# 2892931976/consensus-rs

Measured on AMD Instinct MI355X. Metric: BFT instance-rounds/sec (whole node), N=64 f=21, 1/2/4/8 GPUs; bit-exact, higher is better.
Workload: dtype u64

## Files before the change

### consensus-rs_amd/csrc/bft_common.h

```cpp
#pragma once
#include <stdint.h>

#if defined(__HIPCC__)
#include <hip/hip_runtime.h>
#define BFT_FN __host__ __device__ inline
#else
#define BFT_FN inline
#endif

namespace bft {

struct Params {
    uint32_t n;
    uint32_t seg;
    uint32_t heights;
    uint32_t hcap;
    uint32_t max_ticks;
    uint32_t block_period;
    uint64_t genesis_time;
    uint64_t seed;
    uint32_t thr16;
    uint32_t byz_count;
    uint32_t crash_thr32;
    uint32_t crash_on;
    uint32_t phase_cap;
    uint32_t need_seed;
    uint64_t silent_mask[4];
    uint32_t first_instance;
    uint32_t n_instances;
    uint32_t genesis_seed;
    uint32_t fast;
    const uint8_t* addresses;
    const uint8_t* genesis_hash;
    uint32_t* committed_height;
    uint32_t* flags;
    uint32_t* ticks;
    uint64_t* views;
    uint32_t* rec;
    uint8_t* hash;
    uint64_t* trace;
    uint32_t trace_ticks;
    uint32_t pad1;
    uint64_t* stamps;
    uint64_t* hist;
    uint32_t window_mask;
    uint32_t rows;
    uint32_t* rcs;
    uint32_t q;
    uint32_t nmask;
    uint32_t* resume_flags;
    uint32_t* resume_q;
    uint32_t* resume_hint;
    uint32_t* save;
    uint64_t save_stride;
    uint32_t resume_mode;
    uint32_t seed_le;
    uint32_t backlog_replay;
    uint32_t pad3;
    uint32_t* backlog;
    uint32_t* mlog;
    uint32_t* mlog_n;
    uint32_t mlog_cap;
    uint32_t pad4;
    uint64_t forged[4];
    uint32_t* vsnap;
    uint32_t* votes;
    uint32_t* sfx;
    uint32_t sfx_x0, sfx_rows;
    uint32_t chain_prio;
    uint32_t rcs_k;
    uint32_t* spec;
    uint32_t chain_mode;
    uint32_t chain_grid;
    uint32_t chain_inline;
};
constexpr uint32_t RCS_DEFAULT_K = 16, RCS_MAX_K = 4096;
constexpr uint32_t MLOG_WORDS = 8;
constexpr uint32_t MLOG_FORGED = 1u, MLOG_WILD = 2u, MLOG_EQUIV = 4u, MLOG_OLD = 8u;

constexpr uint32_t FLAG_SAFETY = 1u, FLAG_PHASE_CAP = 2u, FLAG_CORE_PANIC = 4u, FLAG_OUTBOX = 8u,
                   FLAG_TIMEOUT = 16u, FLAG_RCS_OVERFLOW = 32u, FLAG_WINDOW = 64u;
constexpr uint32_t HIST_BINS = 130;
constexpr int NSTAMP = 18;

constexpr uint32_t ST_ACCEPT_REQUEST = 1, ST_PREPREPARED = 2, ST_PREPARED = 3, ST_COMMITTED = 4;

constexpr int MT_PREPREPARE = 1, MT_PREPARE = 2, MT_COMMIT = 3, MT_ROUND_CHANGE = 4;
constexpr int CM_OK = 0, CM_UNKNOWN = 1, CM_FUTURE_BLOCK = 2, CM_OLD = 3, CM_FUTURE_MSG = 4;
BFT_FN int check_message_class(int code, uint32_t vh, uint32_t h, uint32_t st) {
    if (vh == 0) return CM_UNKNOWN;
    if (code == MT_ROUND_CHANGE) { if (vh > h) return CM_FUTURE_BLOCK; if (vh < h) return CM_OLD; return CM_OK; }
    if (vh > h) return CM_FUTURE_BLOCK;
    if (vh < h) return CM_OLD;
    if (st == ST_ACCEPT_REQUEST) return code > MT_PREPREPARE ? CM_FUTURE_MSG : CM_OK;
    return CM_OK;
}

constexpr uint64_t BLK_NONE = 0;
constexpr uint64_t BLK_VALID = 1ull << 34;
constexpr uint64_t BLK_ID_MASK = (1ull << 35) - 1;
constexpr uint64_t BLK_HP_MASK = (1ull << 33) - 1;
BFT_FN uint64_t blk_make(uint32_t h, uint32_t prop, uint32_t var, uint32_t T) {
    return (uint64_t)(h & 0xffffffu) | ((uint64_t)(prop & 0x1ffu) << 24) | ((uint64_t)(var & 1u) << 33) |
           BLK_VALID | ((uint64_t)T << 35);
}
BFT_FN bool blk_valid(uint64_t b) { return (b & BLK_VALID) != 0; }
BFT_FN uint32_t blk_h(uint64_t b) { return (uint32_t)(b & 0xffffffu); }
BFT_FN uint32_t blk_prop(uint64_t b) { return (uint32_t)((b >> 24) & 0x1ffu); }
BFT_FN uint32_t blk_var(uint64_t b) { return (uint32_t)((b >> 33) & 1u); }
BFT_FN uint32_t blk_T(uint64_t b) { return (uint32_t)(b >> 35); }
BFT_FN bool blk_eq(uint64_t a, uint64_t b) {
    return blk_valid(a) && blk_valid(b) && ((a ^ b) & BLK_ID_MASK) == 0;
}
BFT_FN uint32_t blk_d32(uint64_t b) {
    if (!blk_valid(b)) return 0;
    return (uint32_t)(b & 0x3fffffu) | (blk_prop(b) << 22) | (blk_var(b) << 30) | 0x80000000u;
}
BFT_FN bool digest_match(uint64_t d, bool wild, uint64_t t) {
    if (!blk_valid(d) || !blk_valid(t)) return false;
    if (((d ^ t) & BLK_HP_MASK) != 0) return false;
    return wild || blk_var(d) == blk_var(t);
}

template <int NW>
struct Bits {
    uint64_t w[NW];
    BFT_FN static Bits zero() { Bits b; for (int k = 0; k < NW; ++k) b.w[k] = 0; return b; }
    BFT_FN static Bits from(uint64_t x) { Bits b = zero(); b.w[0] = x; return b; }
    BFT_FN static Bits from(const Bits& x) { return x; }
    BFT_FN static Bits low(uint32_t n) {
        if (NW == 1) { Bits b; b.w[0] = n >= 64u ? ~0ull : ((1ull << n) - 1ull); return b; }
        Bits b;
        for (int k = 0; k < NW; ++k) {
            uint32_t lo = 64u * (uint32_t)k;
            b.w[k] = n >= lo + 64u ? ~0ull : (n <= lo ? 0ull : ((1ull << (n - lo)) - 1ull));
        }
        return b;
    }
    BFT_FN static Bits bit(uint32_t i) {
        Bits b;
        for (int k = 0; k < NW; ++k) b.w[k] = ((i >> 6) == (uint32_t)k) ? (1ull << (i & 63u)) : 0ull;
        return b;
    }
    BFT_FN uint64_t word(int i) const {
        uint64_t x = 0;
        for (int k = 0; k < NW; ++k) x = (i == k) ? w[k] : x;
        return x;
    }
    BFT_FN bool get(uint32_t i) const { return (word((int)(i >> 6)) >> (i & 63u)) & 1ull; }
    BFT_FN void set(uint32_t i) {
        const uint64_t b = 1ull << (i & 63u);
        for (int k = 0; k < NW; ++k) w[k] |= ((i >> 6) == (uint32_t)k) ? b : 0ull;
    }
    BFT_FN bool any() const { uint64_t x = 0; for (int k = 0; k < NW; ++k) x |= w[k]; return x != 0; }
    BFT_FN bool none() const { return !any(); }
    BFT_FN uint32_t popc() const {
        uint32_t c = 0;
        for (int k = 0; k < NW; ++k) c += (uint32_t)__builtin_popcountll(w[k]);
// ... 664 lines not shown
```

### consensus-rs_amd/csrc/bftsim.hip

```cpp
#include <hip/hip_runtime.h>

#include <stdio.h>
#include <stdlib.h>
#include <string.h>

#include <dlfcn.h>
#include <unistd.h>
#include <rccl/rccl.h>
#include <hipcub/hipcub.hpp>

#include <mutex>
#include <string>
#include <utility>
#include <vector>

#include "bft_hip.h"
#include "bft_fast64.h"
#include "bft_crypto.h"
#include "bft_trace.h"
#include "bft_twins.h"
#include "bft_audit.h"
#include "bft_archive.h"
#include "bft_ledger.h"

// ... 583 lines not shown
                       (uint32_t*)(h->d_evict + EVICT_BYTES / 16));
    return hipGetLastError();
}

static void use_set0_scratch(bftsim* h) {
    if (h->n_sets == 0 || !h->sets[0].hist) return;
    bftsim::RowSet& r = h->sets[0];
    h->d_hist = r.hist; h->d_rcs = r.rcs; h->d_backlog = r.backlog; h->d_resume = r.resume; h->d_save = r.save;
    h->d_resume_q = r.resume_q;
}

static void trace_drop(bftsim* h) {
    if (!h->d_tkeep && !h->d_tfoff && h->trace_n == 0) return;
    (void)hipFree(h->d_tkeep); (void)hipFree(h->d_tfoff); (void)hipFree(h->d_twkeep);
    h->d_tkeep = nullptr; h->d_tfoff = nullptr; h->d_twkeep = nullptr; h->d_tif0 = nullptr;
    h->trace_n = h->trace_M = h->trace_F = 0;
    h->trace_has_twins = false;
    h->twin_counts[0] = h->twin_counts[1] = 0;
    h->trace_moff.clear(); h->trace_ioff.clear();
}

static int sync_all(bftsim* h);
static void free_bufs(bftsim* h) {
    trace_drop(h);
    if (h->n_pend) (void)sync_all(h);
    h->n_pend = 0;
    h->last_pipe = false;
    use_set0_scratch(h);
    if (h->n_sets == 0) {
        (void)hipFree(h->d_ch); (void)hipFree(h->d_flags); (void)hipFree(h->d_ticks); (void)hipFree(h->d_views);
        (void)hipFree(h->d_rec); (void)hipFree(h->d_hash);
    }
    for (uint32_t k = 0; k < h->n_sets; ++k) {
        bftsim::RowSet& r = h->sets[k];
        (void)hipFree(r.ch); (void)hipFree(r.flags); (void)hipFree(r.ticks); (void)hipFree(r.views);
        (void)hipFree(r.rec); (void)hipFree(r.hash); (void)hipFree(r.sfx); (void)hipFree(r.spec);
        (void)hipFree(r.byz); (void)hipFree(r.bad); (void)hipFree(r.pred);
        if (k > 0) {
            (void)hipFree(r.hist); (void)hipFree(r.rcs); (void)hipFree(r.backlog); (void)hipFree(r.resume);
            (void)hipFree(r.save); (void)hipFree(r.resume_q);
        }
        r.ch = r.flags = r.ticks = nullptr; r.views = nullptr; r.rec = nullptr; r.hash = nullptr; r.sfx = nullptr;
        r.spec = nullptr; r.byz = nullptr; r.bad = nullptr; r.pred = nullptr;
        r.hist = nullptr; r.rcs = r.backlog = r.resume = r.save = r.resume_q = nullptr;
    }

    (void)hipFree(h->d_trace); (void)hipFree(h->d_tips); (void)hipFree(h->d_rcs);
    h->d_rcs = nullptr;
    (void)hipFree(h->d_backlog);
    h->d_backlog = nullptr;
    (void)hipFree(h->d_mlog); (void)hipFree(h->d_mlog_n);
    h->d_mlog = nullptr; h->d_mlog_n = nullptr;
    (void)hipFree(h->d_vsnap); (void)hipFree(h->d_votes); (void)hipFree(h->d_vsig); (void)hipFree(h->d_vhas);
    h->d_vsnap = nullptr; h->d_votes = nullptr; h->d_vsig = nullptr; h->d_vhas = nullptr; h->vsig_n = 0;
    h->backlog_bytes = 0;
    (void)hipFree(h->d_resume); (void)hipFree(h->d_save); (void)hipFree(h->d_resume_q);
    h->d_resume = nullptr; h->d_save = nullptr; h->d_resume_q = nullptr;
    for (uint32_t k = 0; k < bftsim::MAX_SETS; ++k) h->sets[k].busy = false;
    h->n_sets = 0;
    h->cur_set = 0;
    h->d_ch = h->d_flags = h->d_ticks = nullptr; h->d_views = nullptr;
    h->d_rec = nullptr; h->d_hash = nullptr; h->d_trace = nullptr; h->d_tips = nullptr;
    h->cap_inst = 0;
    h->n_req = 0;
    h->last_n = 0;
    h->last_first = 0;
}

static int flush_batch(bftsim* h, bool final = false);
static int sync_all(bftsim* h) {
    HIPCHECK(h, hipSetDevice(h->device));
    if (int rc = flush_batch(h, true)) return rc;
    HIPCHECK(h, hipStreamSynchronize(h->last_stream));
    for (uint32_t k = 0; k < bftsim::MAX_CS; ++k)
        if (h->cs[k]) HIPCHECK(h, hipStreamSynchronize(h->cs[k]));
    for (uint32_t k = 0; k < bftsim::MAX_HS; ++k)
        if (h->hstr[k]) HIPCHECK(h, hipStreamSynchronize(h->hstr[k]));
    return BFTSIM_OK;
}

#ifdef BFT_STAMPS
static uint64_t* g_stamps = nullptr;
static uint64_t g_stamp_waves = 0;
#endif

namespace {
struct Rccl {
    ncclResult_t (*get_id)(ncclUniqueId*) = nullptr;
    ncclResult_t (*init_rank)(ncclComm_t*, int, ncclUniqueId, int) = nullptr;
    ncclResult_t (*all_reduce)(const void*, void*, size_t, ncclDataType_t, ncclRedOp_t, ncclComm_t,
                               hipStream_t) = nullptr;
    ncclResult_t (*destroy)(ncclComm_t) = nullptr;
    const char* (*err)(ncclResult_t) = nullptr;
    bool ok = false;
    std::string why;
};
Rccl& rccl() {
    static Rccl r;
    static std::once_flag once;
    std::call_once(once, [] {
        void* lib = dlopen("librccl.so.1", RTLD_NOW | RTLD_GLOBAL);
        if (!lib) lib = dlopen("/opt/rocm/lib/librccl.so.1", RTLD_NOW | RTLD_GLOBAL);
        if (!lib) { r.why = std::string("dlopen librccl.so.1: ") + dlerror(); return; }
        r.get_id = (decltype(r.get_id))dlsym(lib, "ncclGetUniqueId");
        r.init_rank = (decltype(r.init_rank))dlsym(lib, "ncclCommInitRank");
        r.all_reduce = (decltype(r.all_reduce))dlsym(lib, "ncclAllReduce");
        r.destroy = (decltype(r.destroy))dlsym(lib, "ncclCommDestroy");
        r.err = (decltype(r.err))dlsym(lib, "ncclGetErrorString");
        r.ok = r.get_id && r.init_rank && r.all_reduce && r.destroy && r.err;
        if (!r.ok) r.why = "librccl.so.1 lacks an entry point";
    });
    return r;
}
struct StdoutToStderr {
    int saved;
    StdoutToStderr() {
        fflush(stdout);
        saved = dup(1);
        if (saved >= 0) dup2(2, 1);
    }
    ~StdoutToStderr() {
        fflush(stdout);
        if (saved >= 0) { dup2(saved, 1); close(saved); }
    }
};
void comm_destroy(ncclComm_t c) {
    if (rccl().ok) (void)rccl().destroy(c);
}

struct SigApi {
    int (*create)(int, void**) = nullptr;
    void (*destroy)(void*) = nullptr;
    const char* (*last_error)(const void*) = nullptr;
    int (*secret_to_address)(void*, const uint8_t*, uint64_t, uint8_t*, uint8_t*, uint8_t*, void*) = nullptr;
    int (*sign)(void*, const uint8_t*, const uint32_t*, const uint8_t*, uint64_t, uint8_t*, uint8_t*, void*) = nullptr;
    int (*recover)(void*, const uint8_t*, const uint8_t*, uint64_t, uint8_t*, uint8_t*, uint8_t*, void*) = nullptr;
    bool ok = false;
    std::string why;
};
void sig_api_anchor() {}
SigApi& sig_api() {
    static SigApi a;
    static std::once_flag once;
    std::call_once(once, [] {
        Dl_info di;
        std::string path = "libbftsig.so";
        if (dladdr((void*)&sig_api_anchor, &di) && di.dli_fname) {
            std::string self = di.dli_fname;
            size_t k = self.rfind('/');
            if (k != std::string::npos) path = self.substr(0, k + 1) + "libbftsig.so";
        }
        void* lib = dlopen(path.c_str(), RTLD_NOW | RTLD_GLOBAL);
        if (!lib) { a.why = std::string("dlopen ") + path + ": " + dlerror(); return; }
        a.create = (decltype(a.create))dlsym(lib, "bftsig_create");
        a.destroy = (decltype(a.destroy))dlsym(lib, "bftsig_destroy");
        a.last_error = (decltype(a.last_error))dlsym(lib, "bftsig_last_error");
        a.secret_to_address = (decltype(a.secret_to_address))dlsym(lib, "bftsig_secret_to_address");
        a.sign = (decltype(a.sign))dlsym(lib, "bftsig_sign");
        a.recover = (decltype(a.recover))dlsym(lib, "bftsig_recover");
        a.ok = a.create && a.destroy && a.last_error && a.secret_to_address && a.sign && a.recover;
        if (!a.ok) a.why = path + " lacks an entry point";
    });
    return a;
}
}

extern "C" {

#ifdef BFT_STAMPS
int bftsim_debug_stamps(uint64_t* out, uint32_t cap) {
    if (!out || cap == 0) return bft::NSTAMP;
    std::vector<uint64_t> v(g_stamp_waves * bft::NSTAMP);
    if (hipDeviceSynchronize() != hipSuccess) return -2;
    if (hipMemcpy(v.data(), g_stamps, v.size() * 8, hipMemcpyDeviceToHost) != hipSuccess) return -2;
    const uint32_t m = cap < (uint32_t)bft::NSTAMP ? cap : (uint32_t)bft::NSTAMP;
    for (uint32_t k = 0; k < m; ++k) out[k] = 0;
    for (uint64_t w = 0; w < g_stamp_waves; ++w)
        for (uint32_t k = 0; k < m; ++k) out[k] += v[w * bft::NSTAMP + k];
    return bft::NSTAMP;
}
#endif

uint32_t bftsim_two_thirds_majority(uint32_t n) { return (2u * n) / 3u; }
uint32_t bftsim_seed_from_hash(const uint8_t hash[32], uint32_t n) { return n ? bft::seed_from_hash(hash, n) : 0; }
uint32_t bftsim_seed_from_hash_order(const uint8_t hash[32], uint32_t n, uint32_t order) {
    return n ? bft::seed_from_hash(hash, n, order == BFTSIM_SEED_LE) : 0;
}
uint32_t bftsim_calc_proposer(const uint8_t prev_hash[32], uint32_t n, uint64_t round) {
    if (n == 0) return 0;
    return (uint32_t)(((uint64_t)bft::seed_from_hash(prev_hash, n) + round % n) % n);
}
void bftsim_keccak256(const uint8_t* data, size_t len, uint8_t out[32]) { host_keccak(data, len, out); }
void bftsim_genesis_hash(const bftsim_config* cfg, uint8_t out[32]) { host_genesis_hash(cfg, out); }
int bftsim_check_message(uint32_t code, uint64_t msg_height, uint64_t core_height, uint32_t state) {
    if (code < 1 || code > 4 || state < 1 || state > 4 || msg_height >= (1ull << 32) || core_height >= (1ull << 32))
        return BFTSIM_EINVAL;
    return bft::check_message_class((int)code, (uint32_t)msg_height, (uint32_t)core_height, state);
}
int bftsim_view_cmp(uint64_t h1, uint64_t r1, uint64_t h2, uint64_t r2) {
    if (h1 != h2) return h1 < h2 ? -1 : 1;
    if (r1 != r2) return r1 < r2 ? -1 : 1;
    return 0;
}

const char* bftsim_last_error(bftsim_t* h) { return h ? h->err.c_str() : "null handle"; }

int bftsim_create(const bftsim_config* cfg, int hip_device, bftsim_t** out) {
    if (!cfg || !out) return BFTSIM_EINVAL;
    *out = nullptr;
    if (cfg->n < 1 || cfg->n > 256) return BFTSIM_EUNSUPPORTED;
    if (cfg->heights < 1 || cfg->heights > (1u << 20) || cfg->max_ticks < 1 || cfg->max_ticks > (1u << 28) ||
        !cfg->addresses || cfg->phase_cap < 1 || cfg->phase_cap > 255 || cfg->block_period < 1)
        return BFTSIM_EINVAL;
    for (uint32_t i = 1; i < cfg->n; ++i)
        if (memcmp(cfg->addresses + 20 * (i - 1), cfg->addresses + 20 * i, 20) >= 0) return BFTSIM_EINVAL;
    if (cfg->seed_byte_order > BFTSIM_SEED_LE || cfg->header_encoding != BFTSIM_ENC_RMP_COMPACT ||
        cfg->backlog_mode > BFTSIM_BACKLOG_REPLAY || cfg->reserved != 0)
        return BFTSIM_EINVAL;
    bftsim* h = new bftsim();
    h->cfg = *cfg;
    h->addresses.assign(cfg->addresses, cfg->addresses + 20 * cfg->n);
    h->cfg.addresses = h->addresses.data();
    h->device = hip_device;
    host_genesis_hash(&h->cfg, h->genesis_hash);
    h->genesis_seed = bft::seed_from_hash(h->genesis_hash, cfg->n, cfg->seed_byte_order == BFTSIM_SEED_LE);
    h->seg = bft::segment_size(cfg->n);
    h->hcap = cfg->heights + 64;
    *out = h;
    hipError_t e = hipSetDevice(hip_device);
    if (e != hipSuccess) return fail(h, BFTSIM_EHIP, std::string("hipSetDevice: ") + hipGetErrorString(e));
    HIPCHECK(h, hipMalloc(&h->d_addr, 20 * cfg->n));
    HIPCHECK(h, hipMemcpy(h->d_addr, h->addresses.data(), 20 * cfg->n, hipMemcpyHostToDevice));
    HIPCHECK(h, hipMalloc(&h->d_ghash, 32));
    HIPCHECK(h, hipMemcpy(h->d_ghash, h->genesis_hash, 32, hipMemcpyHostToDevice));
    HIPCHECK(h, hipMalloc(&h->d_stats, 16 * sizeof(unsigned long long)));
    HIPCHECK(h, hipMalloc(&h->d_hist, bft::HIST_BINS * sizeof(uint64_t)));
    for (uint32_t i = 0; i < bftsim::RING; ++i) {
        HIPCHECK(h, hipEventCreate(&h->ring[i].c0)); HIPCHECK(h, hipEventCreate(&h->ring[i].c1));
        HIPCHECK(h, hipEventCreate(&h->ring[i].h0)); HIPCHECK(h, hipEventCreate(&h->ring[i].h1));
        HIPCHECK(h, hipEventCreateWithFlags(&h->ring[i].sx, hipEventDisableTiming));
    }
    for (uint32_t i = 0; i < bftsim::MAX_SETS; ++i)
        HIPCHECK(h, hipEventCreateWithFlags(&h->sets[i].done, hipEventDisableTiming));
    return BFTSIM_OK;
}

void bftsim_destroy(bftsim_t* h) {
    if (!h) return;
    (void)hipSetDevice(h->device);
    free_bufs(h);
    (void)hipFree(h->d_addr); (void)hipFree(h->d_ghash); (void)hipFree(h->d_stats); (void)hipFree(h->d_hist);
    (void)hipFree(h->d_red);
    (void)hipFree(h->d_evict);
    (void)hipFree(h->d_keys);
    if (h->comm) comm_destroy(h->comm);
    if (h->sig) sig_api().destroy(h->sig);
    for (uint32_t i = 0; i < bftsim::RING; ++i) {
        if (h->ring[i].c0) (void)hipEventDestroy(h->ring[i].c0);
        if (h->ring[i].c1) (void)hipEventDestroy(h->ring[i].c1);
        if (h->ring[i].h0) (void)hipEventDestroy(h->ring[i].h0);
        if (h->ring[i].h1) (void)hipEventDestroy(h->ring[i].h1);
        if (h->ring[i].sx) (void)hipEventDestroy(h->ring[i].sx);
// ... 309 lines not shown
                       fast_launch ? h->d_resume_q : nullptr);
    HIPCHECK(h, hipGetLastError());
    if (h->d_backlog) HIPCHECK(h, hipMemsetAsync(h->d_backlog, 0, h->backlog_bytes, s));
    uint32_t per_block = h->seg > 64 ? 1u : 64u / h->seg;
    uint32_t grid = (uint32_t)((n + per_block - 1) / per_block);
    size_t lds = bft::lds_bytes(h->seg, p.need_seed != 0);
    const bool ext = p.backlog_replay || p.mlog;
    HIPCHECK(h, hipEventRecord(ev.c0, s));
    if (fast) {
        p.resume_flags = h->d_resume;
        p.resume_q = h->d_resume_q;
        p.save = h->d_save;
        p.save_stride = n * 64;
        {
            bftsim::RowSet& r = h->sets[pipe ? h->cur_set : 0];
            if (!r.hint) {
                HIPCHECK(h, hipHostMalloc((void**)&r.hint, 4, hipHostMallocMapped | hipHostMallocCoherent));
                *r.hint = 0xffffffffu;
                for (uint32_t k = 0; k < h->n_sets; ++k)
                    if (h->sets[k].hint && &h->sets[k] != &r && *h->sets[k].hint != 0xffffffffu) {
                        *r.hint = __atomic_load_n(h->sets[k].hint, __ATOMIC_RELAXED);
                        break;
                    }
            }
            p.resume_hint = r.hint;
        }
        if (spec) {
            p.spec = h->sets[pipe ? h->cur_set : 0].spec;
            HIPCHECK(h, bft::launch_seed_chain((uint32_t)n, s, p));
            HIPCHECK(h, pmc_evict(h, s));
        }
        HIPCHECK(h, bft::launch_fast(dim3(grid), s, p));
        HIPCHECK(h, pmc_evict(h, s));
        HIPCHECK(h, bft::launch_resume(dim3(grid), lds, s, p));
        HIPCHECK(h, pmc_evict(h, s));
    } else {
        HIPCHECK(h, bft::launch_general(p.need_seed != 0, ext, h->seg, dim3(grid), lds, s, p));
        HIPCHECK(h, pmc_evict(h, s));
    }
    HIPCHECK(h, hipEventRecord(ev.c1, s));
    ev.has_hash = !p.need_seed;
    ev.pending = true;
    if (!p.need_seed) {
        uint32_t* sfx = h->sets[pipe ? h->cur_set : 0].sfx;
        const uint32_t H = h->cfg.heights, K = h->sfx_rows;
        const bool on_launch = fast;
        if (pipe && K >= H && on_launch) {
            bftsim::RowSet& r = h->sets[h->cur_set];
            const bool hspec = r.byz && n < h->hash_spec_max && ((p.thr16 == 0 && p.crash_on == 0) || h->spec_lossy);
            if (!hspec) {
                if (!(h->chain_inline && chain_kind(h, n, false) == bft::CHAIN_KERNEL_LANE)) {
                    HIPCHECK(h, bft::launch_hash_suffix((uint32_t)n, 1, K, sfx, false, s, p));
                    HIPCHECK(h, pmc_evict(h, s));
                }
                HIPCHECK(h, hipEventRecord(ev.sx, s));
            }
            ev.has_hash = false;
            if (h->n_pend > 0 && (h->batch_p.n_instances != p.n_instances || h->batch_spec != hspec))
                if (int rc = flush_batch(h)) return rc;
            if (h->n_pend == 0) {
                h->batch_p = p;
                h->batch_spec = hspec;
                h->cur_hs = (h->cur_hs + 1) % (hspec ? bftsim::N_HS_SPEC : h->n_hs);
                if (!h->hstr[h->cur_hs]) HIPCHECK(h, hipStreamCreateWithFlags(&h->hstr[h->cur_hs], hipStreamNonBlocking));
                h->batch_hs = h->cur_hs;
            }
            h->pend[h->n_pend++] = {h->cur_set, (h->ring_head - 1) % bftsim::RING, (uint32_t)first, h->cur_cs};
            if (h->n_pend >= h->hash_batch) if (int rc = flush_batch(h)) return rc;
        } else {
            hipStream_t t = s;
            if (pipe) {
                h->cur_hs = (h->cur_hs + 1) % h->n_hs;
                if (!h->hstr[h->cur_hs]) HIPCHECK(h, hipStreamCreateWithFlags(&h->hstr[h->cur_hs], hipStreamNonBlocking));
                t = h->hstr[h->cur_hs];
                HIPCHECK(h, hipStreamWaitEvent(t, ev.c1, 0));
            }
            HIPCHECK(h, hipEventRecord(ev.h0, t));
            const uint32_t kind = chain_kind(h, n, false);
            for (uint32_t x0 = 1; x0 <= H; x0 += K) {
                if (!(h->chain_inline && kind == bft::CHAIN_KERNEL_LANE)) {
                    HIPCHECK(h, bft::launch_hash_suffix((uint32_t)n, x0, K, sfx, !on_launch, t, p));
                    HIPCHECK(h, pmc_evict(h, t));
                }
                HIPCHECK(h, bft::launch_hash_chain((uint32_t)n, x0, K, sfx, kind, t, p));
                HIPCHECK(h, pmc_evict(h, t));
            }
            HIPCHECK(h, hipEventRecord(ev.h1, t));
            if (pipe) {
                HIPCHECK(h, hipEventRecord(h->sets[h->cur_set].done, t));
                h->sets[h->cur_set].batch_done = nullptr;
                h->sets[h->cur_set].busy = true;
            }
        }
    }
    if (pipe && p.need_seed) {
        HIPCHECK(h, hipEventRecord(h->sets[h->cur_set].done, s));
        h->sets[h->cur_set].batch_done = nullptr;
        h->sets[h->cur_set].busy = true;
    }
    h->last_n = n;
    h->vsig_n = 0;
    trace_drop(h);
    h->last_first = first;
    h->last_stream = s;
    return BFTSIM_OK;
}

static int flush_batch(bftsim* h, bool final) {
    if (h->n_pend == 0) return BFTSIM_OK;
    hipStream_t t = h->hstr[h->batch_hs];
    const bool conv = final && !h->batch_spec && h->sets[h->pend[0].set].byz != nullptr &&
                      ((h->batch_p.thr16 == 0 && h->batch_p.crash_on == 0) || h->spec_lossy);
    const bool spec = h->batch_spec || conv;
    bft::ChainSets cs{};
    cs.count = h->n_pend;
    int32_t last_on[bftsim::MAX_CS];
    for (uint32_t k = 0; k < bftsim::MAX_CS; ++k) last_on[k] = -1;
    for (uint32_t i = 0; i < h->n_pend; ++i) last_on[h->pend[i].cs] = (int32_t)i;
    if (!spec) {
        for (uint32_t k = 0; k < bftsim::MAX_CS; ++k)
            if (last_on[k] >= 0) HIPCHECK(h, hipStreamWaitEvent(t, h->ring[h->pend[last_on[k]].ev].sx, 0));
    } else {
        HIPCHECK(h, hipStreamWaitEvent(t, h->sets[h->pend[h->n_pend - 1].set].entry, 0));
        hipEvent_t seen[bftsim::MAX_BATCH];
        uint32_t ns = 0;
        for (uint32_t i = 0; i < h->n_pend; ++i) {
            const bftsim::RowSet& r = h->sets[h->pend[i].set];
            if (!r.busy) continue;
            const hipEvent_t e = r.batch_done ? r.batch_done : r.done;
            bool dup = false;
            for (uint32_t j = 0; j < ns; ++j) dup |= seen[j] == e;
            if (dup) continue;
            seen[ns++] = e;
            HIPCHECK(h, hipStreamWaitEvent(t, e, 0));
        }
    }
    for (uint32_t i = 0; i < h->n_pend; ++i) {
        const bftsim::RowSet& r = h->sets[h->pend[i].set];
        cs.sfx[i] = r.sfx; cs.ch[i] = r.ch; cs.hash[i] = r.hash;
        cs.rec[i] = r.rec; cs.byz[i] = r.byz; cs.bad[i] = r.bad; cs.pred[i] = r.pred; cs.first[i] = h->pend[i].first;
    }
    bftsim::LaunchEv& last = h->ring[h->pend[h->n_pend - 1].ev];
    bft::Params p = h->batch_p;
    HIPCHECK(h, hipEventRecord(last.h0, t));
    if (spec) {
        const uint32_t kind = conv ? bft::CHAIN_KERNEL_PAIR : chain_kind(h, p.n_instances, true);
        p.chain_prio = kind == bft::CHAIN_KERNEL_LANE ? bftsim::PRIO_SPEC_LANE : bftsim::PRIO_SPEC_PAIR;
        if (!(kind == bft::CHAIN_KERNEL_LANE && h->chain_inline)) {
            HIPCHECK(h, bft::launch_spec_suffix(p.n_instances, cs, t, p));
            HIPCHECK(h, pmc_evict(h, t));
        }
        p.chain_mode = bft::CHAIN_PREDICTED;
        HIPCHECK(h, bft::launch_hash_chain_batch(p.n_instances, cs, kind, t, p));
        HIPCHECK(h, pmc_evict(h, t));
        for (uint32_t k = 0; k < bftsim::MAX_CS; ++k)
            if (last_on[k] >= 0) HIPCHECK(h, hipStreamWaitEvent(t, h->ring[h->pend[last_on[k]].ev].c1, 0));
        HIPCHECK(h, bft::launch_spec_verify(p.n_instances, cs, t, p));
        HIPCHECK(h, pmc_evict(h, t));
        p.chain_mode = bft::CHAIN_REPAIR;
        HIPCHECK(h, bft::launch_hash_chain_batch(p.n_instances, cs, kind, t, p));
    } else {
        p.chain_mode = bft::CHAIN_RECORDED;
        HIPCHECK(h, bft::launch_hash_chain_batch(p.n_instances, cs, chain_kind(h, p.n_instances, false), t, p));
    }
    HIPCHECK(h, pmc_evict(h, t));
    HIPCHECK(h, hipEventRecord(last.h1, t));
    last.has_hash = true;
    hipEvent_t& bd = h->batch_ev[h->batch_ev_head++ % bftsim::BATCH_EVS];
    if (!bd) HIPCHECK(h, hipEventCreateWithFlags(&bd, hipEventDisableTiming));
    HIPCHECK(h, hipEventRecord(bd, t));
    for (uint32_t i = 0; i < h->n_pend; ++i) {
        bftsim::RowSet& r = h->sets[h->pend[i].set];
        r.batch_done = bd;
        r.busy = true;
    }
    h->n_pend = 0;
    return BFTSIM_OK;
}

int bftsim_set_hash_batch(bftsim_t* h, uint32_t launches) {
    if (!h) return BFTSIM_EINVAL;
    if (launches < 1 || launches > bftsim::MAX_BATCH) return fail(h, BFTSIM_EINVAL, "hash batch must be 1..32 launches");
    if (int rc = flush_batch(h)) return rc;
    h->hash_batch = launches;
    return BFTSIM_OK;
}

int bftsim_set_pipeline(bftsim_t* h, int on) {
    if (!h) return BFTSIM_EINVAL;
    if (on < 0 || on > (int)bftsim::MAX_SETS) return fail(h, BFTSIM_EINVAL, "pipeline depth must be 0..32");
    const int depth = on == 0 ? 0 : on == 1 ? 2 : on;
    if (depth == h->pipeline) return BFTSIM_OK;
    int rc = h->last_stream ? sync_all(h) : BFTSIM_OK;
    if (rc) return rc;
    h->pipeline = depth;
    (void)hipSetDevice(h->device);
    free_bufs(h);
    return BFTSIM_OK;
}

int bftsim_kernel_ms_sum(bftsim_t* h, double* consensus_ms, double* hash_ms, uint32_t* launches) {
    if (!h) return BFTSIM_EINVAL;
    if (int rc = flush_batch(h)) return rc;
    for (uint32_t i = 0; i < bftsim::RING; ++i) {
        bftsim::LaunchEv& ev = h->ring[i];
        if (!ev.pending) continue;
        HIPCHECK(h, hipEventSynchronize(ev.has_hash ? ev.h1 : ev.c1));
        float a = 0, b = 0;
        HIPCHECK(h, hipEventElapsedTime(&a, ev.c0, ev.c1));
        if (ev.has_hash) HIPCHECK(h, hipEventElapsedTime(&b, ev.h0, ev.h1));
        h->acc_c += a; h->acc_h += b; h->acc_n += 1;
        ev.pending = false;
    }
    if (consensus_ms) *consensus_ms = h->acc_c;
    if (hash_ms) *hash_ms = h->acc_h;
    if (launches) *launches = h->acc_n;
    h->acc_c = h->acc_h = 0;
    h->acc_n = 0;
    return BFTSIM_OK;
}

int bftsim_sync(bftsim_t* h) {
    if (!h) return BFTSIM_EINVAL;
    if (!h->last_stream) return BFTSIM_OK;
    return sync_all(h);
}

int bftsim_last_kernel_ms(bftsim_t* h, float* cms, float* hms) {
    if (!h || h->ring_head == 0) return BFTSIM_EINVAL;
    if (int rc = flush_batch(h)) return rc;
    bftsim::LaunchEv& ev = h->ring[(h->ring_head - 1) % bftsim::RING];
    HIPCHECK(h, hipEventSynchronize(ev.has_hash ? ev.h1 : ev.c1));
    float a = 0, b = 0;
    HIPCHECK(h, hipEventElapsedTime(&a, ev.c0, ev.c1));
    if (ev.has_hash) HIPCHECK(h, hipEventElapsedTime(&b, ev.h0, ev.h1));
    if (cms) *cms = a;
    if (hms) *hms = b;
    return BFTSIM_OK;
}

static int check_launched(bftsim* h, uint64_t capacity, const char* what) {
    if (h->last_n == 0 || !h->d_ch) return fail(h, BFTSIM_EINVAL, std::string(what) + ": nothing launched");
    if (capacity < h->last_n)
        return fail(h, BFTSIM_EINVAL, std::string(what) + ": buffers hold " + std::to_string(capacity) +
                                          " instances, the last launch has " + std::to_string(h->last_n));
// ... 1107 lines not shown
```

### consensus-rs_amd/csrc/kern_fast.hip

```cpp
#include "bft_hip.h"
#include "bft_fast64.h"

namespace bft {

#ifndef BFT_FAST_WAVES_PER_SIMD
#define BFT_FAST_WAVES_PER_SIMD 4
#endif
#ifndef BFT_FAST_LOSSLESS_WAVES_PER_SIMD
#define BFT_FAST_LOSSLESS_WAVES_PER_SIMD 4
#endif
#ifndef BFT_FAST_SEEDED_WAVES_PER_SIMD
#define BFT_FAST_SEEDED_WAVES_PER_SIMD 4
#endif
template <bool LOSSY, bool SEEDED>
__global__ __launch_bounds__(64, SEEDED ? BFT_FAST_SEEDED_WAVES_PER_SIMD
                                        : LOSSY ? BFT_FAST_WAVES_PER_SIMD : BFT_FAST_LOSSLESS_WAVES_PER_SIMD)
void bft_consensus_fast_kernel(Params p) {
    extern __shared__ uint8_t lds[];
#ifndef BFT_CONSENSUS_PRIO
#define BFT_CONSENSUS_PRIO 2
#endif
    __builtin_amdgcn_s_setprio(BFT_CONSENSUS_PRIO);
    Fast64<WaveHip, LOSSY, SEEDED> sim(p, lds, blockIdx.x);
    sim.run();
// ... 288 lines not shown
    uint32_t* const pred = predicted ? cs.pred[k] + (uint64_t)il * p.heights : nullptr;
    for (uint32_t x = xs; x <= x1; ++x) {
        const uint32_t rowoff = 4u * il + (x - x0) * SFX_DEV_DW * n4;
        uint32_t len_s;
        if constexpr (INLINE) {
            uint32_t prop, var, tick;
            if (p.chain_mode == CHAIN_PREDICTED) {
                const bool ok = spec_block64(p.seed, cs.first[k] + il, x, byz, 0u, prop, var);
                pred[x - 1u] = ok ? SPEC_VALID | prop | (var << 16) : 0u;
                if (!ok) break;
                tick = x - 1u;
            } else {
                const uint4 row = *(const uint4*)(rec + 4u * x);
                prop = row.y & 0xffffu;
                var = (row.y >> 16) & 1u;
                tick = row.z;
            }
            HdrWriter w(sl, 64u);
            header_suffix_fields(w, p.addresses + 20u * prop, p.seed, cs.first[k] + il, x, prop, var,
                                 p.genesis_time + (uint64_t)p.block_period * ((uint64_t)tick + 1ull));
            len_s = 8u * w.wi + w.fill;
            w.store(w.wi++, w.acc | (0x01ull << (8u * w.fill)));
            while (w.wi < SFX_LDS_DW / 2u) w.store(w.wi++, 0);
        } else {
            len_s = *(const uint32_t*)(sbase + rowoff + SFX_DEV_LEN_DW * n4);
        }
        if (len_s == 0u) break;
        uint32_t pw[2 * PFX_WORDS];
        const uint32_t len_p = header_prefix_regs(prev, ptbl, pw);
        const uint32_t c = 72u - len_p, r = c & 3u, nb = splice_blocks(len_p, len_s);
        const int j0 = (int)(c >> 2) - (int)SFX_PAD;
        auto G = [&](uint32_t jj) -> uint32_t {
            if constexpr (INLINE) return sl[64u * jj];
            else return *(const uint32_t*)(sbase + rowoff + __umul24(jj, n4));
        };
        constexpr int BODY = INLINE ? (int)SFX_LDS_DW : (int)SFX_BODY_DW;
        auto S = [&](int j) -> uint32_t {
            const uint32_t v = G((uint32_t)(j < 0 ? 0 : j > BODY - 1 ? BODY - 1 : j));
            return ((j >= 0) & (j < BODY)) ? v : 0u;
        };
        uint32_t L[25], H[25];
#pragma unroll
        for (int i = 0; i < 25; ++i) {
            L[i] = i < (int)PFX_WORDS ? pw[2 * i] : 0u;
            H[i] = i < (int)PFX_WORDS ? pw[2 * i + 1] : 0u;
        }
        for (uint32_t blk = 0; blk < nb; ++blk) {
            uint32_t d[35];
            if (blk == 0u) {
#pragma unroll
                for (int i = 0; i < 17; ++i) d[i] = S(j0 + i);
                if constexpr (INLINE) {
#pragma unroll
                    for (int i = 17; i < 35; ++i) d[i] = G((uint32_t)(j0 + i));
                } else {
                    uint32_t vo = rowoff + __umul24((uint32_t)(j0 + 17), n4);
#pragma unroll
                    for (int i = 17; i < 35; ++i, vo += n4) d[i] = *(const uint32_t*)(sbase + vo);
                }
#pragma unroll
                for (int i = 0; i < 34; ++i) d[i] = align_bytes(d[i + 1], d[i], r);
            } else {
#pragma unroll
                for (int i = 0; i < 35; ++i) d[i] = S(j0 + 34 * (int)blk + i);
#pragma unroll
                for (int i = 0; i < 34; ++i) d[i] = align_bytes(d[i + 1], d[i], r);
            }
#pragma unroll
            for (int i = 0; i < 17; ++i) { L[i] ^= d[2 * i]; H[i] ^= d[2 * i + 1]; }
            if (blk + 1u == nb) H[16] ^= 0x80000000u;
            keccak_f1600_lane(L, H);
        }
        uint32_t* dst = (uint32_t*)(hash + ((uint64_t)il * p.rows + x) * 32);
#pragma unroll
        for (int i = 0; i < 4; ++i) { prev[2 * i] = L[i]; prev[2 * i + 1] = H[i]; }
        *(uint4*)dst = make_uint4(prev[0], prev[1], prev[2], prev[3]);
        *(uint4*)(dst + 4) = make_uint4(prev[4], prev[5], prev[6], prev[7]);
    }
}
#endif
#ifndef BFT_LANE_WAVES_PER_SIMD
#define BFT_LANE_WAVES_PER_SIMD 4
#endif

template <bool INLINE>
__global__ __launch_bounds__(64, INLINE ? BFT_LANE_WAVES_PER_SIMD : 3) void bft_hash_chain_lane_kernel(Params p, ChainSets cs) {
#if defined(__HIP_DEVICE_COMPILE__)
    set_prio(p.chain_prio);
    __shared__ PfxSel ptbl[16];
    extern __shared__ uint32_t sfx_lds[];
    if (threadIdx.x < 16) ptbl[threadIdx.x] = PFX_TBL[threadIdx.x];
    __syncthreads();
    const uint32_t bps = (p.n_instances + 63u) / 64u, tasks = cs.count * bps;
    for (uint32_t t = blockIdx.x; t < tasks; t += gridDim.x) {
        const uint32_t k = t / bps, il = (t % bps) * 64u + threadIdx.x;
        if (il < p.n_instances)
            lane_chain<INLINE>(p, cs, k, il, ptbl, INLINE ? sfx_lds + threadIdx.x : nullptr);
    }
#endif
}
static hipError_t launch_lane(uint32_t tasks, const ChainSets& cs, hipStream_t s, const Params& p) {
    const uint32_t g = p.chain_grid && p.chain_grid < tasks ? p.chain_grid : tasks;
    if (p.chain_inline)
        hipLaunchKernelGGL(bft_hash_chain_lane_kernel<true>, dim3(g), dim3(64), (size_t)SFX_LDS_DW * 64u * 4u, s, p, cs);
    else hipLaunchKernelGGL(bft_hash_chain_lane_kernel<false>, dim3(g), dim3(64), 0, s, p, cs);
    return hipGetLastError();
}

__global__ __launch_bounds__(256) void bft_spec_byz_kernel(Params p, ChainSets cs) {
    set_prio(p.chain_prio);
    __shared__ uint8_t perm[256 * 64];
    const uint32_t n = p.n_instances, bpl = (n + 255u) / 256u, k = blockIdx.x / bpl;
    const uint32_t il = (blockIdx.x % bpl) * 256u + threadIdx.x;
    if (il >= n) return;
    cs.byz[k][il] = byz_mask64(p.seed, cs.first[k] + il, p.byz_count, perm + 64u * threadIdx.x);
    cs.bad[k][il] = 0xffffffffu;
}
__device__ inline uint64_t spec_time(const Params& p, uint32_t tick) {
    return p.genesis_time + (uint64_t)p.block_period * ((uint64_t)tick + 1ull);
}
__global__ __launch_bounds__(256) void bft_spec_suffix_kernel(Params p, ChainSets cs) {
    set_prio(p.chain_prio);
    const uint32_t n = p.n_instances, H = p.heights;
    const uint32_t bpl = (uint32_t)(((uint64_t)n * H + 255u) / 256u), k = blockIdx.x / bpl;
    const uint32_t t = (blockIdx.x % bpl) * 256u + threadIdx.x;
    const uint32_t j = t / n, il = t - j * n;
    if (j >= H) return;
    const uint32_t x = j + 1u, inst = cs.first[k] + il;
    uint32_t* row = const_cast<uint32_t*>(cs.sfx[k]) + (uint64_t)j * SFX_DEV_DW * n + il;
    uint32_t prop, var;
    if (!spec_block64(p.seed, inst, x, cs.byz[k][il], 0u, prop, var)) {
        row[(uint64_t)SFX_DEV_LEN_DW * n] = 0u;
        cs.pred[k][(uint64_t)il * H + j] = 0u;
        return;
    }
    cs.pred[k][(uint64_t)il * H + j] = SPEC_VALID | prop | (var << 16);
    header_suffix_strided(row, n, p.addresses + 20u * prop, p.seed, inst, x, prop, var, spec_time(p, x - 1u));
}
__global__ __launch_bounds__(256) void bft_spec_verify_kernel(Params p, ChainSets cs) {
    const uint32_t n = p.n_instances, H = p.heights;
    const uint32_t bpl = (uint32_t)(((uint64_t)n * H + 255u) / 256u), k = blockIdx.x / bpl;
    const uint32_t t = (blockIdx.x % bpl) * 256u + threadIdx.x;
    const uint32_t il = t / H, x = t - il * H + 1u;
    if (il >= n) return;
    if (x > cs.ch[k][il]) return;
    const uint4 row = *(const uint4*)(cs.rec[k] + ((uint64_t)il * p.rows + x) * 4);
    const uint32_t pw = cs.pred[k][(uint64_t)il * H + x - 1u], inst = cs.first[k] + il;
    if (((pw & SPEC_VALID) != 0u) & ((row.y & 0x1ffffu) == (pw & 0x1ffffu)) & (row.z + 1u == x)) return;
    const uint32_t rp = row.y & 0xffffu, rv = (row.y >> 16) & 1u;
    header_suffix_strided(const_cast<uint32_t*>(cs.sfx[k]) + (uint64_t)(x - 1u) * SFX_DEV_DW * n + il, n,
                          p.addresses + 20u * rp, p.seed, inst, x, rp, rv, spec_time(p, row.z));
    atomicMin(&cs.bad[k][il], x);
}
hipError_t launch_spec_suffix(uint32_t n, const ChainSets& cs, hipStream_t s, const Params& p) {
    if (cs.count < 1 || cs.count > CHAIN_MAX_SETS || p.n_instances != n) return hipErrorInvalidValue;
    hipLaunchKernelGGL(bft_spec_byz_kernel, dim3(cs.count * ((n + 255u) / 256u)), dim3(256), 0, s, p, cs);
    const uint32_t bpl = (uint32_t)(((uint64_t)n * p.heights + 255u) / 256u);
    hipLaunchKernelGGL(bft_spec_suffix_kernel, dim3(cs.count * bpl), dim3(256), 0, s, p, cs);
    return hipGetLastError();
}
hipError_t launch_spec_verify(uint32_t n, const ChainSets& cs, hipStream_t s, const Params& p) {
    if (cs.count < 1 || cs.count > CHAIN_MAX_SETS || p.n_instances != n) return hipErrorInvalidValue;
    const uint32_t bpl = (uint32_t)(((uint64_t)n * p.heights + 255u) / 256u);
    hipLaunchKernelGGL(bft_spec_verify_kernel, dim3(cs.count * bpl), dim3(256), 0, s, p, cs);
    return hipGetLastError();
}

__global__ __launch_bounds__(CHAIN_PAIR_BLOCK) void bft_seed_chain_kernel(Params p) {
#if defined(__HIP_DEVICE_COMPILE__)
    __shared__ __attribute__((aligned(16))) uint32_t sbuf[32 * CHAIN_SB];
    __shared__ __attribute__((aligned(16))) uint64_t pbuf[CHAIN_PB_SLOTS * (PFX_WORDS + 4)];
    __shared__ PfxSel ptbl[16];
    __shared__ uint32_t slen[32];
    if (threadIdx.x < 16) ptbl[threadIdx.x] = PFX_TBL[threadIdx.x];
    __syncthreads();
    const uint32_t odd = threadIdx.x & 1u, pair = threadIdx.x >> 1;
    const uint32_t il = blockIdx.x * 32u + pair;
    if (il >= p.n_instances) return;
    const uint32_t n = p.n_instances, inst = p.first_instance + il;
    uint32_t* sb = sbuf + pair * CHAIN_SB;
    const uint64_t byz = byz_mask64(p.seed, inst, p.byz_count, (uint8_t*)(sb + SFX_PAD) + 64u * odd);
    __syncthreads();
    for (uint32_t i = odd; i < SFX_PAD; i += 2u) sb[i] = 0;
    for (uint32_t i = SFX_PAD + SFX_BODY_DW + odd; i < CHAIN_SB; i += 2u) sb[i] = 0;
    const uint8_t* ph = p.genesis_hash;
    uint32_t prev[8];
    for (int i = 0; i < 8; ++i)
        prev[i] = (uint32_t)ph[4 * i] | ((uint32_t)ph[4 * i + 1] << 8) | ((uint32_t)ph[4 * i + 2] << 16) |
// ... 91 lines not shown
```

Measured before the change: 3.493 billion.

## Pack multiple lane-chain waves per workgroup and add chain timing records

The hash-chain lane kernel now launches workgroups of four 64-lane waves instead of one wave per block. Each wave takes its own task index and its own LDS suffix slice, and the grid shrinks by the same factor. This cuts the number of workgroup dispatches and the per-block PFX table setup, at the cost of larger LDS per block, which may limit how many blocks fit per CU. It also adds optional per-wave timing records, compiled only under BFT_STAMPS, for profiling chain work placement.

```diff
diff --git a/consensus-rs_amd/csrc/bft_common.h b/consensus-rs_amd/csrc/bft_common.h
--- a/consensus-rs_amd/csrc/bft_common.h
+++ b/consensus-rs_amd/csrc/bft_common.h
@@ -73,7 +73,11 @@
     uint32_t chain_mode;
     uint32_t chain_grid;
     uint32_t chain_inline;
+#ifdef BFT_STAMPS
+    uint32_t stamp_seq;
+#endif
 };
+constexpr uint32_t CHAIN_REC_HDR = 2, CHAIN_REC_WORDS = 4;
 constexpr uint32_t RCS_DEFAULT_K = 16, RCS_MAX_K = 4096;
 constexpr uint32_t MLOG_WORDS = 8;
 constexpr uint32_t MLOG_FORGED = 1u, MLOG_WILD = 2u, MLOG_EQUIV = 4u, MLOG_OLD = 8u;
diff --git a/consensus-rs_amd/csrc/bftsim.hip b/consensus-rs_amd/csrc/bftsim.hip
--- a/consensus-rs_amd/csrc/bftsim.hip
+++ b/consensus-rs_amd/csrc/bftsim.hip
@@ -689,6 +689,24 @@
 #ifdef BFT_STAMPS
 static uint64_t* g_stamps = nullptr;
 static uint64_t g_stamp_waves = 0;
+static uint64_t* g_chain_rec = nullptr;
+static uint32_t g_chain_seq = 0;
+static constexpr uint64_t CHAIN_REC_CAP = 1u << 16;
+static hipError_t chain_rec_arm(bft::Params& p) {
+    if (!g_chain_rec) {
+        const size_t bytes = (bft::CHAIN_REC_HDR + CHAIN_REC_CAP * bft::CHAIN_REC_WORDS) * 8;
+        if (hipError_t e = hipMalloc(&g_chain_rec, bytes)) return e;
+        const uint64_t hdr[bft::CHAIN_REC_HDR] = {0, CHAIN_REC_CAP};
+        if (hipError_t e = hipMemset(g_chain_rec, 0, bytes)) return e;
+        if (hipError_t e = hipMemcpy(g_chain_rec, hdr, sizeof hdr, hipMemcpyHostToDevice)) return e;
+    }
+    p.stamps = g_chain_rec;
+    p.stamp_seq = g_chain_seq++;
+    return hipSuccess;
+}
+#define CHAIN_REC_ARM(h, p) HIPCHECK(h, chain_rec_arm(p))
+#else
+#define CHAIN_REC_ARM(h, p) do { } while (0)
 #endif
 
 namespace {
@@ -785,6 +803,18 @@
     for (uint64_t w = 0; w < g_stamp_waves; ++w)
         for (uint32_t k = 0; k < m; ++k) out[k] += v[w * bft::NSTAMP + k];
     return bft::NSTAMP;
+}
+int64_t bftsim_debug_chain_records(uint64_t* out, uint32_t cap_records, int reset) {
+    if (hipDeviceSynchronize() != hipSuccess) return -2;
+    if (!g_chain_rec) return 0;
+    uint64_t hdr[bft::CHAIN_REC_HDR];
+    if (hipMemcpy(hdr, g_chain_rec, sizeof hdr, hipMemcpyDeviceToHost) != hipSuccess) return -2;
+    uint64_t m = hdr[0] < CHAIN_REC_CAP ? hdr[0] : CHAIN_REC_CAP;
+    if (m > cap_records) m = cap_records;
+    if (out && m && hipMemcpy(out, g_chain_rec + bft::CHAIN_REC_HDR, m * bft::CHAIN_REC_WORDS * 8,
+                              hipMemcpyDeviceToHost) != hipSuccess) return -2;
+    if (reset && hipMemset(g_chain_rec, 0, 8) != hipSuccess) return -2;
+    return (int64_t)hdr[0];
 }
 #endif
 
@@ -1260,6 +1290,7 @@
                     HIPCHECK(h, bft::launch_hash_suffix((uint32_t)n, x0, K, sfx, !on_launch, t, p));
                     HIPCHECK(h, pmc_evict(h, t));
                 }
+                CHAIN_REC_ARM(h, p);
                 HIPCHECK(h, bft::launch_hash_chain((uint32_t)n, x0, K, sfx, kind, t, p));
                 HIPCHECK(h, pmc_evict(h, t));
             }
@@ -1329,6 +1360,7 @@
             HIPCHECK(h, pmc_evict(h, t));
         }
         p.chain_mode = bft::CHAIN_PREDICTED;
+        CHAIN_REC_ARM(h, p);
         HIPCHECK(h, bft::launch_hash_chain_batch(p.n_instances, cs, kind, t, p));
         HIPCHECK(h, pmc_evict(h, t));
         for (uint32_t k = 0; k < bftsim::MAX_CS; ++k)
@@ -1336,9 +1368,11 @@
         HIPCHECK(h, bft::launch_spec_verify(p.n_instances, cs, t, p));
         HIPCHECK(h, pmc_evict(h, t));
         p.chain_mode = bft::CHAIN_REPAIR;
+        CHAIN_REC_ARM(h, p);
         HIPCHECK(h, bft::launch_hash_chain_batch(p.n_instances, cs, kind, t, p));
     } else {
         p.chain_mode = bft::CHAIN_RECORDED;
+        CHAIN_REC_ARM(h, p);
         HIPCHECK(h, bft::launch_hash_chain_batch(p.n_instances, cs, chain_kind(h, p.n_instances, false), t, p));
     }
     HIPCHECK(h, pmc_evict(h, t));
diff --git a/consensus-rs_amd/csrc/kern_fast.hip b/consensus-rs_amd/csrc/kern_fast.hip
--- a/consensus-rs_amd/csrc/kern_fast.hip
+++ b/consensus-rs_amd/csrc/kern_fast.hip
@@ -394,28 +394,68 @@
 #ifndef BFT_LANE_WAVES_PER_SIMD
 #define BFT_LANE_WAVES_PER_SIMD 4
 #endif
+#ifndef BFT_LANE_GROUP_WAVES
+#define BFT_LANE_GROUP_WAVES 4
+#endif
+constexpr uint32_t LANE_GROUP_WAVES = BFT_LANE_GROUP_WAVES;
+
+#if defined(BFT_STAMPS) && defined(__HIP_DEVICE_COMPILE__)
+struct ChainStamp { uint64_t t0; uint32_t hw, xcc; };
+__device__ inline ChainStamp chain_stamp_begin() {
+    ChainStamp s;
+    s.hw = __builtin_amdgcn_s_getreg(4 | (31 << 11));
+    s.xcc = __builtin_amdgcn_s_getreg(20 | (31 << 11));
+    s.t0 = __builtin_amdgcn_s_memrealtime();
+    return s;
+}
+__device__ inline void chain_stamp_end(const Params& p, const ChainStamp& s, uint32_t task) {
+    if ((threadIdx.x & 63u) != 0u || !p.stamps) return;
+    const uint64_t t1 = __builtin_amdgcn_s_memrealtime();
+    const uint64_t i = atomicAdd((unsigned long long*)p.stamps, 1ull);
+    if (i >= p.stamps[1]) return;
+    uint64_t* r = p.stamps + CHAIN_REC_HDR + CHAIN_REC_WORDS * i;
+    r[0] = (uint64_t)s.hw | ((uint64_t)(s.xcc & 15u) << 32) | ((uint64_t)(threadIdx.x >> 6) << 36) |
+           ((uint64_t)(p.stamp_seq & 0xffffffu) << 40);
+    r[1] = s.t0;
+    r[2] = t1;
+    r[3] = (uint64_t)task | ((uint64_t)(blockIdx.x & 0xfffffffu) << 32) | ((uint64_t)(p.chain_mode & 3u) << 60);
+}
+#endif
 
 template <bool INLINE>
-__global__ __launch_bounds__(64, INLINE ? BFT_LANE_WAVES_PER_SIMD : 3) void bft_hash_chain_lane_kernel(Params p, ChainSets cs) {
+__global__ __launch_bounds__(64 * LANE_GROUP_WAVES, INLINE ? BFT_LANE_WAVES_PER_SIMD : 3)
+void bft_hash_chain_lane_kernel(Params p, ChainSets cs) {
 #if defined(__HIP_DEVICE_COMPILE__)
     set_prio(p.chain_prio);
+#ifdef BFT_STAMPS
+    const ChainStamp stamp = chain_stamp_begin();
+#endif
     __shared__ PfxSel ptbl[16];
     extern __shared__ uint32_t sfx_lds[];
     if (threadIdx.x < 16) ptbl[threadIdx.x] = PFX_TBL[threadIdx.x];
     __syncthreads();
+    const uint32_t wave = __builtin_amdgcn_readfirstlane(threadIdx.x >> 6), lane = threadIdx.x & 63u;
+    uint32_t* const sl = INLINE ? sfx_lds + wave * (SFX_LDS_DW * 64u) + lane : nullptr;
     const uint32_t bps = (p.n_instances + 63u) / 64u, tasks = cs.count * bps;
-    for (uint32_t t = blockIdx.x; t < tasks; t += gridDim.x) {
-        const uint32_t k = t / bps, il = (t % bps) * 64u + threadIdx.x;
-        if (il < p.n_instances)
-            lane_chain<INLINE>(p, cs, k, il, ptbl, INLINE ? sfx_lds + threadIdx.x : nullptr);
-    }
+    constexpr uint32_t GW = LANE_GROUP_WAVES;
+    const uint32_t t0 = GW * blockIdx.x + wave;
+    for (uint32_t t = t0; t < tasks; t += GW * gridDim.x) {
+        const uint32_t k = t / bps, il = (t % bps) * 64u + lane;
+        if (il < p.n_instances) lane_chain<INLINE>(p, cs, k, il, ptbl, sl);
+    }
+#ifdef BFT_STAMPS
+    chain_stamp_end(p, stamp, t0);
+#endif
 #endif
 }
 static hipError_t launch_lane(uint32_t tasks, const ChainSets& cs, hipStream_t s, const Params& p) {
-    const uint32_t g = p.chain_grid && p.chain_grid < tasks ? p.chain_grid : tasks;
+    constexpr uint32_t GW = LANE_GROUP_WAVES;
+    const uint32_t waves = p.chain_grid && p.chain_grid < tasks ? p.chain_grid : tasks;
+    const uint32_t g = (waves + GW - 1u) / GW;
     if (p.chain_inline)
-        hipLaunchKernelGGL(bft_hash_chain_lane_kernel<true>, dim3(g), dim3(64), (size_t)SFX_LDS_DW * 64u * 4u, s, p, cs);
-    else hipLaunchKernelGGL(bft_hash_chain_lane_kernel<false>, dim3(g), dim3(64), 0, s, p, cs);
+        hipLaunchKernelGGL(bft_hash_chain_lane_kernel<true>, dim3(g), dim3(64u * GW),
+                           (size_t)GW * SFX_LDS_DW * 64u * 4u, s, p, cs);
+    else hipLaunchKernelGGL(bft_hash_chain_lane_kernel<false>, dim3(g), dim3(64u * GW), 0, s, p, cs);
     return hipGetLastError();
 }
 
```

Result: no change. 3.465 billion (-0.8%).
